# VUmcCGP/wisecondor

Measured on AMD Instinct MI355X. Metric: newref bin-pair distances/sec, higher is better.
Workload: dtype f64; 1 GPU; cfg2: newref 100 samples x 250 kb bins (11087 masked bins, refsize 100); parallelism=newref sharded by single rank, symmetric tiles, 1 rank(s), world_size=1

## Files before the change

### wisecondor_amd/csrc/ctx.h

```cpp
#pragma once
#include "common.h"

#define WC_MAX_CHROM 64

struct NewrefState {
    int64_t n_bins = 0, n_samples = 0;
    int64_t bins_pad = 0;
    int64_t k_pad16 = 0;
    int n_chrom = 0, k = 0, sum_order = 0;
    int64_t chrom_off[WC_MAX_CHROM + 1] = {0};
    const double *corrected = nullptr;
    int64_t n_sample_cols = 0;
    int64_t cap = 0;
    int64_t expect = 0;
    float beta = 0.f;
    bool prepared = false;
    double tau = 0.0;
    wc::DevBuf col_partial, col_mean, norm_lo, norm_hi, chrom_of_row, chrom_range, chrom_off_dev;
    wc::DevBuf sample_rows, sample_slot, s32, s_norm_lo, s_chrom, s_range, a16, s16;
    wc::DevBuf keys1, thr, cnt, list, tiles;
    wc::DevBuf fb_rows, fb_count, fb_scratch, stats, tiles0, pw_prog, pairs, x64, m2;
    bool fb_dirty = true;
    int64_t s_pad = 0;
    bool exact_only = false;
    wc::DevBuf cand_word;
    int index_bits = 17;
    int index_bits_req = 0;
    bool x64_pad = false;
    int pw_leaves = 0;
    int64_t pw_for = -1;
    std::vector<int64_t> sample_key, tiles0_key, tiles1_key, chrom_key;
    int64_t tiles0_n = 0, tiles1_n = 0;
};

struct TestState {
    std::vector<int> sel_host;
    wc::DevBuf counts, totals, raw, proj, data, xt, xc, zt, rt, nt, sdt, z, r, n, sd_avg;
    wc::DevBuf zc, rc, gpos, regions, sel;
    wc::DevBuf res_z, res_r, cwz, calls, n_calls;
    wc::DevBuf zs, rs2, ns2, sds, sub, tmin, tmax, tmin2, tmax2, cell_state, cell_rec, prefix, reg_abs, reg_flag, rs, jobs_a, jobs_b, job_cnt, partial, cbound, cuts, job_res, hot, cand, cand_cnt;
    wc::DevBuf seg, out_val, out_x, out_y, out_n, whole, effect, misc, misc2, reduce_tmp, win_bits, bit_off, pairs_a, pairs_b, cut_vals;
    wc::DevBuf walk_hot;
    int64_t rs_len = 0;
    hipGraphExec_t lat_exec = nullptr;
    std::vector<int64_t> lat_key, lat_fail_key;
    bool lat_warm = false;
    unsigned long long lat_epoch = 0;
    bool profile = false;
    std::vector<hipEvent_t> prof_ev;
    std::vector<int> prof_tag;
    wc::DevBuf sd_fail;
    wc::DevBuf prof_work;
    void mark(int tag, hipStream_t stream) {
        if (!profile) return;
        const size_t at = prof_tag.size();
        if (at >= prof_ev.size()) {
            hipEvent_t e = nullptr;
            if (hipEventCreate(&e) != hipSuccess) return;
            prof_ev.push_back(e);
        }
        if (hipEventRecord(prof_ev[at], stream) == hipSuccess) prof_tag.push_back(tag);
    }
};

struct PrepState {
    int64_t S = 0, Btot = 0, B = 0;
    bool ready = false;
    wc::DevBuf eig_ws;
};

struct ConvertState {
    wc::DevBuf tab, tiles, kpos, cls;
};

struct wc_ctx {
    int device = 0;
    PrepState prep;
    ConvertState cv;
    NewrefState nr;
    TestState ts;
    wc::DevBuf tmp_a, tmp_b, tmp_c, tmp_d;
    wc::DevBuf df_scratch, df_meta;
    wc::DevBuf js_slots, js_tiles;
    wc::DevBuf sp_plan;
    wc::DevBuf pl_list, pl_counts, pl_tab, pl_img, pl_part, pl_status;
    unsigned char *pl_host = nullptr;
    size_t pl_host_bytes = 0;
    hipEvent_t pl_sent = nullptr;
    int pl_host_reserve(size_t bytes) {
        if (!pl_sent) WC_HIP(hipEventCreateWithFlags(&pl_sent, hipEventDisableTiming));
        else WC_HIP(hipEventSynchronize(pl_sent));
        if (bytes <= pl_host_bytes) return WC_OK;
        if (pl_host) (void)hipHostFree(pl_host);
        pl_host = nullptr;
        pl_host_bytes = 0;
        const size_t ask = bytes + (bytes >> 1) + 256;
        WC_HIP(hipHostMalloc((void **)&pl_host, ask, hipHostMallocDefault));
        pl_host_bytes = ask;
        return WC_OK;
    }
    void *pinned = nullptr;
    size_t pinned_bytes = 0;
    int64_t last_stats[8] = {0};
    hipStream_t lat_stream = nullptr;
    hipEvent_t ev_lat_in = nullptr, ev_lat_out = nullptr;
// ... 73 lines not shown
```

### wisecondor_amd/csrc/newref.hip

```cpp
#include <cstring>
#include "ctx.h"

#include <algorithm>
#include <stdlib.h>

namespace {

constexpr int TB = 128;
constexpr int BK = 32;
constexpr int LDA = 36;
constexpr int LDT = 68;
constexpr int ROLE_ROWS = 1;
constexpr int ROLE_COLS = 2;
constexpr int MAX_SAMPLE_COLS = 4096;
constexpr int LIST_CAP = 1024;
constexpr int K_MAX = 1024;
constexpr int GL_ROW = 16;
constexpr int GL_STAGE = 2 * TB * GL_ROW;
#define WC_ADMIT_ALL FLT_MAX
constexpr double SENTINEL_DISTANCE = 1e10;

typedef float f32x16 __attribute__((ext_vector_type(16)));
typedef float f32x4 __attribute__((ext_vector_type(4)));
typedef _Float16 f16x8 __attribute__((ext_vector_type(8)));
// ... 2 lines not shown
typedef unsigned long long u64x2 __attribute__((ext_vector_type(2)));
typedef __attribute__((address_space(3))) void lds_void_t;
typedef __attribute__((address_space(1))) const void glb_void_t;
typedef __attribute__((address_space(3))) char lds_char_t;
typedef __attribute__((address_space(3))) f64x2 lds_f64x2_t;

__global__ __launch_bounds__(1024) void k_col_centre(const double *__restrict__ X, int64_t B, int64_t S,
                                                     int64_t n_rows, int64_t row_step,
                                                     double *__restrict__ centre, int *__restrict__ bad_norm) {
    __shared__ double sh_s[16][64];
    __shared__ double sh_c[16][64];
    __shared__ double sh_v[64];
    const int tx = threadIdx.x & 63, ty = threadIdx.x >> 6;
    const int64_t s = (int64_t)blockIdx.x * 64 + tx;
    if (blockIdx.x == 0 && threadIdx.x == 0) *bad_norm = 0x7F800000;
    constexpr int PER = 8;
    double val[PER];
#pragma unroll
    for (int e = 0; e < PER; ++e) {
        const int64_t q = ty + 16 * e;
        val[e] = (s < S && q < n_rows) ? X[(q * row_step) * S + s] : NAN;
    }
    double c = 0.0, rad = 0.0;
    for (int pass = 0; pass < 3; ++pass) {
        double sum = 0.0, cnt = 0.0;
#pragma unroll
        for (int e = 0; e < PER; ++e) {
            const double v = val[e];
            const bool ok = isfinite(v) && (pass != 2 || fabs(v - c) <= rad);
            sum += ok ? ((pass == 1) ? fabs(v - c) : v) : 0.0;
            cnt += ok ? 1.0 : 0.0;
        }
        sh_s[ty][tx] = sum;
        sh_c[ty][tx] = cnt;
        wc_sync();
        if (ty == 0) {
            double a = 0.0, b = 0.0;
            for (int r = 0; r < 16; ++r) { a += sh_s[r][tx]; b += sh_c[r][tx]; }
            sh_v[tx] = b > 0.0 ? a / b : 0.0;
        }
        wc_sync();
        if (pass == 0) c = sh_v[tx];
        else if (pass == 1) {
            rad = 8.0 * sh_v[tx];
            if (ty == 0 && s < S) centre[S + s] = sh_v[tx];
        } else if (ty == 0 && s < S) centre[s] = sh_v[tx];
        wc_sync();
    }
}

__device__ __host__ inline int64_t a16_index(int64_t row, int64_t s, int64_t Kpad16) {
    return (((row >> 7) * (Kpad16 >> 5) + (s >> 5)) << 12) + ((row & 127) << 5) + (s & 31);
}

__device__ inline unsigned short f32_to_f16_scaled(float a, double gam, double inv_gam, double &back, bool &clamped) {
    double sd = (double)a * gam;
    clamped = clamped || sd > 65504.0 || sd < -65504.0;
    sd = sd > 65504.0 ? 65504.0 : (sd < -65504.0 ? -65504.0 : sd);
    _Float16 h = (_Float16)(float)sd;
    if (fabs((double)(float)h) < 6.103515625e-05) h = (_Float16)0.f;
    back = (double)(float)h * inv_gam;
    unsigned short bits;
    __builtin_memcpy(&bits, &h, 2);
    return bits;
}

__host__ __device__ inline unsigned int slack_encode(float slack, int cb) {
    unsigned int u;
    __builtin_memcpy(&u, &slack, 4);
    u = u > 0x7F800000u ? 0x7F800000u : u;
    const int sh = 31 - cb;
    return (u + ((1u << sh) - 1u)) >> sh;
}
__host__ __device__ inline float slack_decode(unsigned int code, int cb) {
    const unsigned int u = code << (31 - cb);
    float f;
    __builtin_memcpy(&f, &u, 4);
    return f;
}
__device__ __forceinline__ float slack_of_word(unsigned int word, unsigned int index_mask) {
    return __uint_as_float((word >> 1) & ~(index_mask >> 1));
}

__global__ __launch_bounds__(256) void k_convert(const double *__restrict__ X, int64_t B, int64_t S,
                                                 int64_t Bpad,
                                                 const double *__restrict__ mean, double beta, double tau,
                                                 const int64_t *__restrict__ chrom_off, int n_chrom,
                                                 unsigned short *__restrict__ A16,
                                                 int64_t Kpad16, float *__restrict__ norm_lo,
                                                 float *__restrict__ norm_hi, int *__restrict__ chrom_of_row,
                                                 int2 *__restrict__ chrom_range,
                                                 const int *__restrict__ sample_slot,
                                                 unsigned short *__restrict__ S16, float *__restrict__ s_norm_lo,
                                                 int *__restrict__ s_chrom, int2 *__restrict__ s_range,
                                                 float *__restrict__ thr, int *__restrict__ cnt,
                                                 int *__restrict__ row_stat,
                                                 double *__restrict__ X64, int64_t Sp, float *__restrict__ m2_out,
                                                 int *__restrict__ bad_norm, int *__restrict__ fb_zero, int n_fb_zero,
                                                 unsigned int *__restrict__ cand_word, int index_bits) {
    const int lane = threadIdx.x & 63, hl = lane & 31, half = lane >> 5;
    const int64_t row = ((int64_t)blockIdx.x * 4 + (threadIdx.x >> 6)) * 2 + half;
    if (blockIdx.x == 0)
        for (int i = threadIdx.x; i < n_fb_zero; i += 256) fb_zero[i] = 0;
    if (row >= Bpad) return;
    constexpr int CB = 4;
    const int64_t xrow = (row < B ? row : 0) * S;
    auto load_x = [&](int64_t s0, double (&xv)[CB], double (&mv)[CB]) {
#pragma unroll
        for (int j = 0; j < CB; ++j) {
            const int64_t s = s0 + 32 * j, sc = s < S ? s : 0;
            xv[j] = X[xrow + sc];
            mv[j] = mean[sc];
        }
    };
    auto pin = [&](double (&v)[CB]) {
#pragma unroll
        for (int j = 0; j < CB; ++j) asm volatile("" : "+v"(v[j]));
    };
    auto load_scale = [&](int64_t s0, double (&sv)[CB]) {
#pragma unroll
        for (int j = 0; j < CB; ++j) {
            const int64_t s = s0 + 32 * j;
            sv[j] = mean[S + (s < S ? s : 0)];
        }
    };
    double xv[CB], mv[CB], sv[CB];
    load_scale(hl, sv);
    load_x(hl, xv, mv);
    int slot_w = sample_slot[row < B ? row : 0];
    int64_t end0_w = chrom_off[hl < n_chrom ? hl + 1 : 0], end1_w = chrom_off[hl + 32 < n_chrom ? hl + 33 : 0];
    asm volatile("" : "+v"(slot_w), "+v"(end0_w), "+v"(end1_w));
    pin(sv);
    pin(xv);
    pin(mv);
    const int slot = row < B ? slot_w : -1;
    int ch_w = -1;
    int2 range_w = make_int2(0, 0);
    {
        const int64_t none = (int64_t)0x7FFFFFFFFFFFFFFFll;
        const int64_t end0 = hl < n_chrom ? end0_w : none, end1 = hl + 32 < n_chrom ? end1_w : none;
        const unsigned long long b0 = __ballot(row < B && hl < n_chrom - 1 && row >= end0);
        const unsigned long long b1 = __ballot(row < B && hl + 32 < n_chrom - 1 && row >= end1);
        const int c = __popc((unsigned int)(b0 >> (32 * half))) + __popc((unsigned int)(b1 >> (32 * half)));
        auto end_of = [&](int i) {
            const int64_t a0 = __shfl(end0, (lane & 32) + (i & 31)), a1 = __shfl(end1, (lane & 32) + (i & 31));
            return i < 32 ? a0 : a1;
        };
        const int64_t e_lo = end_of(c ? c - 1 : 0), e_hi = end_of(c);
        if (row < B) {
            ch_w = c;
            range_w = make_int2((int)(c ? e_lo : 0), (int)e_hi);
        }
    }
    double gam = 1.0, inv_gam = 1.0;
    {
        double t = 0.0, c = 0.0;
        for (int64_t s0 = hl; s0 < S; s0 += 32 * CB) {
            if (s0 != hl) { load_scale(s0, sv); pin(sv); }
#pragma unroll
            for (int j = 0; j < CB; ++j) {
                const double m = sv[j];
                if (s0 + 32 * j < S && isfinite(m) && m > 0.0) { t += m; c += 1.0; }
            }
        }
        for (int o = 16; o > 0; o >>= 1) { t += __shfl_xor(t, o); c += __shfl_xor(c, o); }
        if (c > 0.0 && isfinite(t)) {
            int e = ilogb(t / c);
            e = e < -60 ? -60 : (e > 60 ? 60 : e);
            gam = ldexp(1.0, 2 - e);
            inv_gam = ldexp(1.0, e - 2);
        }
        if (row == 0 && hl == 0) *m2_out = (float)(-2.0 * inv_gam * inv_gam);
    }
    double acc = 0.0, e2 = 0.0, hn = 0.0;
    bool clamped = false;
    for (int64_t s0 = hl; s0 < Kpad16; s0 += 32 * CB) {
        if (s0 != hl) { load_x(s0, xv, mv); pin(xv); pin(mv); }
#pragma unroll
        for (int j = 0; j < CB; ++j) {
            const int64_t s = s0 + 32 * j;
            if (s < Kpad16) {
                if (X64 && row < B && s < Sp) X64[row * Sp + s] = s < S ? xv[j] : 0.0;
                float a = 0.f;
                if (row < B && s < S) a = (float)(xv[j] - mv[j]);
                double back;
                const unsigned short h = f32_to_f16_scaled(a, gam, inv_gam, back, clamped);
                const double err = (double)a - back;
                e2 += err * err;
                hn += back * back;
                A16[a16_index(row, s, Kpad16)] = h;
                if (slot >= 0) S16[(int64_t)slot * Kpad16 + s] = h;
                acc += (double)a * (double)a;
            }
        }
    }
    for (int o = 16; o > 0; o >>= 1) {
        acc += __shfl_xor(acc, o);
        e2 += __shfl_xor(e2, o);
        hn += __shfl_xor(hn, o);
    }
    clamped = ((unsigned int)(__ballot(clamped) >> (32 * half))) != 0u;
    if (hl == 0) {
        float lo = INFINITY, hi = INFINITY;
        int ch = -1;
        int2 range = make_int2(0, 0);
        if (row < B) {
            if (isfinite(acc) && acc < 1e37 && isfinite(e2) && isfinite(hn) && clamped) {
                atomicMin(bad_norm, __float_as_int(__double2float_rd(sqrt(acc) * (1.0 - 1e-6))));
            } else if (isfinite(acc) && acc < 1e37 && isfinite(e2) && isfinite(hn)) {
                const double m = fmax(acc, hn);
                lo = __double2float_rd(acc - (e2 / tau + tau * m) * (1.0 + 1e-9) - beta * m - 1e-37);
                hi = __double2float_ru(2.0 * (acc - (double)lo) * (1.0 + 1e-6) + 1e-37);
            }
            ch = ch_w;
            range = range_w;
        }
        chrom_range[row] = range;
        norm_lo[row] = lo;
        norm_hi[row] = hi;
        cand_word[row] = (unsigned int)row | (slack_encode(hi, 32 - index_bits) << index_bits);
        chrom_of_row[row] = ch;
        if (slot >= 0) {
            s_norm_lo[slot] = lo;
            s_chrom[slot] = ch;
            s_range[slot] = range;
        }
        thr[row] = -INFINITY;
        cnt[row] = 0;
        row_stat[row] = (int)0xFEFEFEFE;
    }
}

__global__ void k_pad_samples(int64_t Kpad16, int64_t first, unsigned short *__restrict__ S16,
                              float *__restrict__ s_norm_lo, int *__restrict__ s_chrom,
                              int2 *__restrict__ s_range) {
    int64_t m = first + blockIdx.x;
    for (int64_t s = threadIdx.x; s < Kpad16; s += blockDim.x) S16[m * Kpad16 + s] = (unsigned short)0;
    if (threadIdx.x == 0) {
        s_norm_lo[m] = INFINITY;
        s_chrom[m] = -2;
        s_range[m] = make_int2(0, 0);
    }
}


struct GramArgs {
    const float *P, *Q;
    int64_t ld;
    const float *m2;
    int nslab32, last_steps32;
    const float *nbP, *nbQ;
    const unsigned int *cwP, *cwQ;
    const int2 *range;
    const int4 *tiles;
    int ntiles;
    const float *thr;
    int *cnt;
    unsigned long long *list;
    int cap;
};

__device__ inline unsigned int key_code16(float key) {
    const unsigned int code = __float_as_uint(fmaxf(key, 0.f)) >> 15;
    return key < INFINITY ? code : 0xFFFFu;
}
__device__ inline float key_from_code16(unsigned int code) {
    return __uint_as_float((code << 15) | 0x7FFFu);
}

__device__ inline unsigned int run_mask(int a, int b) {
    a = a < 0 ? 0 : a;
    b = b > 32 ? 32 : b;
    if (a >= b) return 0u;
    const unsigned int upto_b = b == 32 ? ~0u : ((1u << b) - 1u);
    return upto_b & ~((1u << a) - 1u);
}

__device__ inline unsigned long long pack_passed(float key, unsigned int word) {
    const unsigned int b = __float_as_uint(key);
    return ((unsigned long long)((b & 0x80000000u) ? ~b : (b | 0x80000000u)) << 32) | word;
}

__device__ __forceinline__ void shift_in_le(unsigned int &mask, float key, float thr) {
    asm("v_cmp_le_f32 vcc, %1, %2\n\tv_addc_co_u32 %0, vcc, %0, %0, vcc" : "+v"(mask) : "v"(key), "v"(thr) : "vcc");
}

__device__ inline void wave_lds_fence() {
    __builtin_amdgcn_fence(__ATOMIC_RELEASE, "wavefront");
    __builtin_amdgcn_wave_barrier();
    __builtin_amdgcn_fence(__ATOMIC_ACQUIRE, "wavefront");
}

__device__ inline unsigned long long pack_entry(float key, int j) {
    return ((unsigned long long)wc::f32_ordered(key) << 32) | (unsigned int)j;
}


constexpr int EP_LD = 32;
constexpr int EP_BLOCK = 64 * EP_LD;
constexpr int EP_MASKS = 128;
static_assert(4 * EP_BLOCK <= 2 * GL_STAGE, "the four dot blocks alias the two operand stages");

__device__ __forceinline__ int ep_at(int col, int row) {
    return col * EP_LD + ((((row >> 2) ^ col) & 7) << 2) + (row & 3);
}

__device__ __forceinline__ void gram_epilogue(const GramArgs &g, float *sm, const float *nbPs, const float *nbQs,
                                              const float *thPs, const float *thQs, const unsigned int *cwPs,
                                              const unsigned int *cwQs, f32x16 (&acc)[2][2], const int I,
                                              const int J, const int roles, const float m2, const int lane, const int w,
                                              const int wr, const int wc, const int li, const int lh) {
    __builtin_amdgcn_s_setprio(0);
    const int row0 = I * TB + wr * 64, col0 = J * TB + wc * 64;
    const int2 rgq0 = g.range[(int64_t)col0 + li], rgq1 = g.range[(int64_t)col0 + 32 + li];
    const int2 rgr = g.range[(int64_t)row0 + lane];
// ... 1706 lines not shown
                 (long long)st.bins_pad, need);
        st.index_bits = st.index_bits_req ? st.index_bits_req : std::min(24, std::max(17, need));
    }
    st.k_pad16 = round_up(n_samples, 64);
    st.cap = LIST_CAP;
    st.expect = LIST_CAP * 3 / 8;
    const double chain = (double)(n_samples + 16) * 5.9604644775390625e-08;
    st.beta = (float)(2.0 * chain * 1.001);
    st.tau = 2.44140625e-04;
    int64_t M = round_up((n_bins + 13) / 14, TB);
    if (M < 512) M = 512;
    if (M > MAX_SAMPLE_COLS) M = MAX_SAMPLE_COLS;
    if (M > st.bins_pad) M = st.bins_pad;
    st.n_sample_cols = M;

    int rc;
    if ((rc = st.col_mean.reserve(sizeof(double) * 3 * n_samples))) return rc;
    st.s_pad = round_up(n_samples, 16);
    st.x64_pad = n_samples <= 2048 && st.bins_pad * st.s_pad * 8 < (1ll << 32);
    if (st.x64_pad && (rc = st.x64.reserve(sizeof(double) * st.bins_pad * st.s_pad))) return rc;
    if ((rc = st.m2.reserve(sizeof(float) * 4))) return rc;
    if ((rc = st.norm_lo.reserve(sizeof(float) * st.bins_pad))) return rc;
    if ((rc = st.norm_hi.reserve(sizeof(float) * st.bins_pad))) return rc;
    if ((rc = st.cand_word.reserve(sizeof(unsigned int) * st.bins_pad))) return rc;
    if ((rc = st.chrom_of_row.reserve(sizeof(int) * st.bins_pad))) return rc;
    if ((rc = st.chrom_range.reserve(sizeof(int2) * st.bins_pad))) return rc;
    if ((rc = st.chrom_off_dev.reserve(sizeof(int64_t) * (WC_MAX_CHROM + 1)))) return rc;
    if ((rc = st.sample_rows.reserve(sizeof(int) * M))) return rc;
    if ((rc = st.sample_slot.reserve(sizeof(int) * st.bins_pad))) return rc;
    if ((rc = st.a16.reserve(sizeof(unsigned short) * st.bins_pad * st.k_pad16))) return rc;
    if ((rc = st.s16.reserve(sizeof(unsigned short) * M * st.k_pad16))) return rc;
    if ((rc = st.s_norm_lo.reserve(sizeof(float) * M))) return rc;
    if ((rc = st.s_chrom.reserve(sizeof(int) * M))) return rc;
    if ((rc = st.s_range.reserve(sizeof(int2) * M))) return rc;
    if ((rc = st.keys1.reserve(sizeof(unsigned short) * st.bins_pad * M))) return rc;
    if ((rc = st.thr.reserve(sizeof(float) * st.bins_pad))) return rc;
    if ((rc = st.cnt.reserve(sizeof(int) * st.bins_pad))) return rc;
    if ((rc = st.list.reserve(sizeof(uint64_t) * st.bins_pad * st.cap))) return rc;
    if ((rc = st.fb_rows.reserve(sizeof(int) * st.bins_pad))) return rc;
    if ((rc = st.fb_count.reserve(sizeof(int) * 4))) return rc;
    if ((rc = st.stats.reserve(sizeof(int) * st.bins_pad))) return rc;

    {
        std::vector<int64_t> ckey(st.chrom_off, st.chrom_off + n_chrom + 1);
        if (ckey != st.chrom_key) {
            WC_HIP(hipMemcpyAsync(st.chrom_off_dev.p, st.chrom_off, sizeof(int64_t) * (n_chrom + 1),
                                  hipMemcpyHostToDevice, stream));
            WC_HIP(hipStreamSynchronize(stream));
            st.chrom_key = ckey;
        }
    }
    if (st.pw_for != n_samples) {
        std::vector<int2> prog;
        build_pairwise_leaves((int)n_samples, 0, prog);
        if ((rc = st.pw_prog.reserve(sizeof(int2) * prog.size()))) return rc;
        WC_HIP(hipMemcpyAsync(st.pw_prog.p, prog.data(), sizeof(int2) * prog.size(), hipMemcpyHostToDevice, stream));
        WC_HIP(hipStreamSynchronize(stream));
        st.pw_leaves = (int)prog.size();
        st.pw_for = n_samples;
    }
    std::vector<int64_t> skey = {n_bins, M};
    if (skey != st.sample_key) {
        int64_t real = std::min<int64_t>(M, n_bins);
        std::vector<int> perm(n_bins);
        for (int64_t i = 0; i < n_bins; ++i) perm[i] = (int)i;
        uint64_t s = 0x9E3779B97F4A7C15ull;
        for (int64_t i = 0; i < real; ++i) {
            s = s * 6364136223846793005ull + 1442695040888963407ull;
            int64_t pick = i + (int64_t)((s >> 33) % (uint64_t)(n_bins - i));
            std::swap(perm[i], perm[pick]);
        }
        std::sort(perm.begin(), perm.begin() + real);
        std::vector<int> slot((size_t)n_bins, -1);
        for (int64_t i = 0; i < real; ++i) slot[perm[i]] = (int)i;
        WC_HIP(hipMemcpyAsync(st.sample_rows.p, perm.data(), sizeof(int) * real, hipMemcpyHostToDevice, stream));
        WC_HIP(hipMemcpyAsync(st.sample_slot.p, slot.data(), sizeof(int) * n_bins, hipMemcpyHostToDevice, stream));
        WC_HIP(hipStreamSynchronize(stream));
        st.sample_key = skey;
        st.tiles0_key.clear();
        st.tiles1_key.clear();
    }

    double *mean2 = st.col_mean.as<double>();
    {
        int64_t n_rows = std::min<int64_t>(n_bins, 128);
        int64_t row_step = n_bins / n_rows;
        hipLaunchKernelGGL(k_col_centre, dim3((unsigned)((n_samples + 63) / 64)), dim3(1024), 0, stream, corrected,
                           n_bins, n_samples, n_rows, row_step, mean2, st.m2.as<int>() + 1);
    }

    hipLaunchKernelGGL(k_convert, dim3((unsigned)(st.bins_pad / 8)), dim3(256), 0, stream, corrected, n_bins,
                       n_samples, st.bins_pad, (const double *)mean2, (double)st.beta, st.tau,
                       st.chrom_off_dev.as<int64_t>(), n_chrom, st.a16.as<unsigned short>(),
                       st.k_pad16, st.norm_lo.as<float>(), st.norm_hi.as<float>(), st.chrom_of_row.as<int>(),
                       st.chrom_range.as<int2>(), (const int *)st.sample_slot.as<int>(),
                       st.s16.as<unsigned short>(), st.s_norm_lo.as<float>(), st.s_chrom.as<int>(),
                       st.s_range.as<int2>(), st.thr.as<float>(), st.cnt.as<int>(), st.stats.as<int>(),
                       st.x64_pad ? st.x64.as<double>() : (double *)nullptr, st.s_pad, st.m2.as<float>(),
                       st.m2.as<int>() + 1, st.fb_count.as<int>(), 4, st.cand_word.as<unsigned int>(), st.index_bits);
    st.fb_dirty = false;
    if (M > n_bins)
        hipLaunchKernelGGL(k_pad_samples, dim3((unsigned)(M - n_bins)), dim3(256), 0, stream, st.k_pad16, n_bins,
                           st.s16.as<unsigned short>(), st.s_norm_lo.as<float>(), st.s_chrom.as<int>(),
                           st.s_range.as<int2>());
    WC_HIP(hipGetLastError());
    st.prepared = true;
    return WC_OK;
}

int wc_newref_thresholds_dev(wc_ctx *ctx, void *stream_, int64_t row_begin, int64_t row_end) {
    WC_CHECK(ctx && ctx->nr.prepared, WC_E_ARG, "newref: prepare has not run");
    NewrefState &st = ctx->nr;
    WC_CHECK(row_begin >= 0 && row_begin <= row_end && row_end <= st.n_bins, WC_E_ARG, "newref: bad row range");
    if (row_begin == row_end || st.exact_only) return WC_OK;
    hipStream_t stream = (hipStream_t)stream_;
    const int ib = (int)(row_begin / TB), ie = (int)((row_end + TB - 1) / TB);
    const int mb = (int)(st.n_sample_cols / TB);
    std::vector<int64_t> key = {st.bins_pad, st.n_sample_cols, ib, ie};
    if (key != st.tiles0_key) {
        std::vector<int4> tiles;
        tiles.reserve((size_t)(ie - ib) * mb);
        for (int I = ib; I < ie; ++I)
            for (int J = 0; J < mb; ++J) tiles.push_back(make_int4(I, J, 0, 0));
        int rc;
        if ((rc = st.tiles0.reserve(sizeof(int4) * tiles.size()))) return rc;
        WC_HIP(hipMemcpyAsync(st.tiles0.p, tiles.data(), sizeof(int4) * tiles.size(), hipMemcpyHostToDevice, stream));
        WC_HIP(hipStreamSynchronize(stream));
        st.tiles0_key = key;
        st.tiles0_n = (int64_t)tiles.size();
    }
    {
        const int ntiles = (int)st.tiles0_n;
        unsigned grid = (unsigned)(((ntiles + 7) / 8) * 8);
        hipLaunchKernelGGL(k_gram_thr16, dim3(grid), dim3(256), 0, stream,
                           (const unsigned short *)st.a16.as<unsigned short>(),
                           (const unsigned short *)st.s16.as<unsigned short>(), st.k_pad16, (int)(st.k_pad16 / 64),
                           (const float *)st.norm_lo.as<float>(), (const float *)st.s_norm_lo.as<float>(),
                           (const int2 *)st.s_range.as<int2>(), (const int4 *)st.tiles0.as<int4>(), ntiles,
                           st.keys1.as<unsigned int>(), st.n_sample_cols, (const float *)st.m2.as<float>());
    }
    unsigned sg = (unsigned)((row_end - row_begin + 3) / 4);
    {
        const unsigned int *kp = st.keys1.as<unsigned int>();
        const int2 *cr = st.chrom_range.as<int2>();
        const int per_lane = (int)(st.n_sample_cols / 64);
#define WC_SELECT(NV)                                                                                          \
    hipLaunchKernelGGL(k_select_thr<NV>, dim3(sg), dim3(256), 0, stream, kp, st.n_sample_cols,                \
                       (int)st.n_sample_cols, cr, st.n_bins, row_begin, row_end, (int)st.expect, (int)st.cap, \
                       st.thr.as<float>())
        if (per_lane <= 16) WC_SELECT(16);
        else if (per_lane <= 32) WC_SELECT(32);
        else WC_SELECT(64);
#undef WC_SELECT
    }
    WC_HIP(hipGetLastError());
    return WC_OK;
}

int64_t wc_newref_list_capacity(wc_ctx *ctx) { return ctx ? ctx->nr.cap : 0; }

int wc_newref_get_thresholds_dev(wc_ctx *ctx, void *stream, int64_t row_begin, int64_t row_end, float *out) {
    WC_CHECK(ctx && ctx->nr.prepared && out, WC_E_ARG, "newref: bad argument");
    WC_CHECK(row_begin >= 0 && row_begin <= row_end && row_end <= ctx->nr.n_bins, WC_E_ARG, "newref: bad row range");
    if (row_end > row_begin)
        WC_HIP(hipMemcpyAsync(out, ctx->nr.thr.as<float>() + row_begin, sizeof(float) * (row_end - row_begin),
                              hipMemcpyDeviceToDevice, (hipStream_t)stream));
    return WC_OK;
}

int wc_newref_get_bounds_dev(wc_ctx *ctx, void *stream, int64_t row_begin, int64_t row_end, float *lo_out,
                             float *slack_out) {
    WC_CHECK(ctx && ctx->nr.prepared && lo_out && slack_out, WC_E_ARG, "newref: bad argument");
    WC_CHECK(row_begin >= 0 && row_begin <= row_end && row_end <= ctx->nr.n_bins, WC_E_ARG, "newref: bad row range");
    if (row_end > row_begin) {
        WC_HIP(hipMemcpyAsync(lo_out, ctx->nr.norm_lo.as<float>() + row_begin, sizeof(float) * (row_end - row_begin),
                              hipMemcpyDeviceToDevice, (hipStream_t)stream));
        WC_HIP(hipMemcpyAsync(slack_out, ctx->nr.norm_hi.as<float>() + row_begin, sizeof(float) * (row_end - row_begin),
                              hipMemcpyDeviceToDevice, (hipStream_t)stream));
    }
    return WC_OK;
}

// ... 54 lines not shown
                               const int32_t *src_cnt, const uint64_t *src_list) {
    WC_CHECK(ctx && ctx->nr.prepared && src_cnt && src_list && src_cap > 0, WC_E_ARG, "newref: bad argument");
    WC_CHECK(row_begin >= 0 && row_begin <= row_end && row_end <= ctx->nr.n_bins, WC_E_ARG, "newref: bad row range");
    if (row_end == row_begin) return WC_OK;
    NewrefState &st = ctx->nr;
    hipLaunchKernelGGL(k_import_lists, dim3((unsigned)(row_end - row_begin)), dim3(64), 0, (hipStream_t)stream,
                       st.cnt.as<int>(), st.list.as<unsigned long long>(), (int)st.cap, row_begin, (int)src_cap,
                       src_cnt, (const unsigned long long *)src_list,
                       (const unsigned int *)st.cand_word.as<unsigned int>(), (1u << st.index_bits) - 1u,
                       (unsigned int)st.bins_pad);
    WC_HIP(hipGetLastError());
    return WC_OK;
}

int wc_newref_collect_dev(wc_ctx *ctx, void *stream_, int64_t row_begin, int64_t row_end, int tile_rank,
                          int tile_ranks) {
    WC_CHECK(ctx && ctx->nr.prepared, WC_E_ARG, "newref: prepare has not run");
    NewrefState &st = ctx->nr;
    WC_CHECK(row_begin >= 0 && row_begin <= row_end && row_end <= st.n_bins, WC_E_ARG, "newref: bad row range");
    WC_CHECK(tile_ranks >= 1 && tile_rank >= 0 && tile_rank < tile_ranks, WC_E_ARG, "newref: bad tile rank");
    if (row_begin == row_end || st.exact_only) return WC_OK;
    hipStream_t stream = (hipStream_t)stream_;
    std::vector<int64_t> key = {st.n_bins, row_begin, row_end, tile_rank, tile_ranks};
    for (int c = 0; c <= st.n_chrom; ++c) key.push_back(st.chrom_off[c]);
    if (key != st.tiles1_key) {
        std::vector<int4> tiles;
        build_tiles(st, row_begin, row_end, tile_rank, tile_ranks, tiles);
        int rc;
        if ((rc = st.tiles.reserve(sizeof(int4) * std::max<size_t>(tiles.size(), 1)))) return rc;
        if (!tiles.empty()) {
            WC_HIP(hipMemcpyAsync(st.tiles.p, tiles.data(), sizeof(int4) * tiles.size(), hipMemcpyHostToDevice, stream));
            WC_HIP(hipStreamSynchronize(stream));
        }
        st.tiles1_key = key;
        st.tiles1_n = (int64_t)tiles.size();
    }
    ctx->last_stats[2] = st.tiles1_n;
    ctx->last_stats[3] = st.n_sample_cols;
    if (st.tiles1_n == 0) return WC_OK;
    GramArgs g{};
    g.P = g.Q = st.a16.as<float>();
    g.ld = st.k_pad16 / 2;
    g.m2 = st.m2.as<float>();
    g.nslab32 = (int)((st.n_samples + 31) / 32);
    g.last_steps32 = (int)(((st.n_samples - (int64_t)(g.nslab32 - 1) * 32) + 15) / 16);
    g.nbP = g.nbQ = st.norm_lo.as<float>();
    g.cwP = g.cwQ = st.cand_word.as<unsigned int>();
    g.range = st.chrom_range.as<int2>();
    g.tiles = st.tiles.as<int4>();
    g.ntiles = (int)st.tiles1_n;
    g.thr = st.thr.as<float>();
    g.cnt = st.cnt.as<int>();
    g.list = st.list.as<unsigned long long>();
    g.cap = (int)st.cap;
    const unsigned grid = (unsigned)(((g.ntiles + 7) / 8) * 8);
    hipLaunchKernelGGL(k_gram_glds, dim3(grid), dim3(256), 0, stream, g);
    WC_HIP(hipGetLastError());
    return WC_OK;
}

static void finish_args(NewrefState &st, int64_t row_begin, int64_t row_end, int32_t *idx_out, double *dist_out,
                        FinishArgs &a) {
    a.X = st.corrected;
    a.B = st.n_bins;
    a.S = st.n_samples;
    a.norm_lo = st.norm_lo.as<float>();
    a.norm_hi = st.norm_hi.as<float>();
    a.thr = st.thr.as<float>();
    a.cnt = st.cnt.as<int>();
    a.list = st.list.as<unsigned long long>();
    a.index_mask = (1u << st.index_bits) - 1u;
    a.cap = (int)st.cap;
    a.k = st.k;
    a.beta = (double)st.beta;
    a.chrom_of_row = st.chrom_of_row.as<int>();
    a.chrom_off = st.chrom_off_dev.as<int64_t>();
    a.chrom_range = st.chrom_range.as<int2>();
    a.row_begin = row_begin;
    a.row_end = row_end;
    a.idx_out = idx_out;
    a.dist_out = dist_out;
    a.fb_rows = st.fb_rows.as<int>();
    a.fb_count = st.fb_count.as<int>();
    a.bad_norm = st.m2.as<float>() + 1;
    a.row_stat = st.stats.as<int>();
    a.sum_order = st.sum_order;
    a.lone_mask = 0ull;
    if (st.sum_order == WC_SUM_SEQUENTIAL)
        for (int c = 0; c < st.n_chrom; ++c)
            if (st.chrom_off[c] <= 1 && st.n_bins - st.chrom_off[c + 1] <= 1) a.lone_mask |= 1ull << c;
    a.xs_in_lds = st.n_samples <= 2048;
    a.pw_prog = st.pw_prog.as<int2>();
    a.pw_leaves = st.pw_leaves;
}

static int launch_exact(NewrefState &st, hipStream_t stream, const FinishArgs &a, int64_t n_host) {
    int rc;
    const int cap = n_host < 0 ? EX_DEV_CAP : EX_CAP;
    if ((rc = st.fb_scratch.reserve(sizeof(uint64_t) * (n_host < 0 ? 2 : 1) * cap * st.bins_pad))) return rc;
    const bool seq = st.sum_order == WC_SUM_SEQUENTIAL || st.n_samples < 8;
    const int edge = seq ? 64 : 32;
    const unsigned ctiles = (unsigned)((st.n_bins + edge - 1) / edge);
    unsigned long long *scratch = st.fb_scratch.as<unsigned long long>();
    const int *rows = st.fb_rows.as<int>();
    if (n_host < 0) {
        const int rgroups = 4;
        int *sync = st.fb_count.as<int>() + 1;
        constexpr int EXD_TILE_WGS = 192, EXD_SEL_WGS = 64;
        const int n_tile = (int)std::min<int64_t>((int64_t)ctiles * rgroups, EXD_TILE_WGS);
        const unsigned grid = (unsigned)(n_tile + EXD_SEL_WGS);
        if (seq) hipLaunchKernelGGL((k_exact_dev<true>), dim3(grid), dim3(256), 0, stream, a, rows,
                                    (const int *)st.fb_count.as<int>(), sync, scratch, st.bins_pad, cap, (int)ctiles, rgroups, EXD_SEL_WGS);
        else hipLaunchKernelGGL((k_exact_dev<false>), dim3(grid), dim3(256), 0, stream, a, rows,
                                (const int *)st.fb_count.as<int>(), sync, scratch, st.bins_pad, cap, (int)ctiles, rgroups, EXD_SEL_WGS);
        return WC_OK;
    }
    for (int64_t first = 0; first < n_host; first += cap) {
        const int64_t nf = std::min<int64_t>(cap, n_host - first);
        const unsigned rgroups = (unsigned)((nf + edge - 1) / edge);
        if (seq) hipLaunchKernelGGL((k_exact_tile<true>), dim3(ctiles, rgroups), dim3(256), 0, stream, a, rows,
                                    (const int *)nullptr, (int)n_host, (int)first, scratch, st.bins_pad, cap);
        else hipLaunchKernelGGL((k_exact_tile<false>), dim3(ctiles, rgroups), dim3(256), 0, stream, a, rows,
                                (const int *)nullptr, (int)n_host, (int)first, scratch, st.bins_pad, cap);
        hipLaunchKernelGGL(k_exact_select, dim3((unsigned)nf), dim3(256), 0, stream, a, rows, (int)n_host, (int)first,
                           scratch, st.bins_pad, cap);
    }
    return WC_OK;
}

static int newref_finish_part(wc_ctx *ctx, void *stream_, int64_t row_begin, int64_t row_end, int32_t *idx_out,
                              double *dist_out, int which) {
    WC_CHECK(ctx && ctx->nr.prepared, WC_E_ARG, "newref: prepare has not run");
    NewrefState &st = ctx->nr;
    WC_CHECK(row_begin >= 0 && row_begin <= row_end && row_end <= st.n_bins, WC_E_ARG, "newref: bad row range");
    WC_CHECK(idx_out && dist_out, WC_E_ARG, "newref: NULL output");
    if (row_begin == row_end) return WC_OK;
    hipStream_t stream = (hipStream_t)stream_;
    int rc;
    if (which & 5) {
        if (st.fb_dirty) WC_HIP(hipMemsetAsync(st.fb_count.p, 0, sizeof(int) * 4, stream));
        st.fb_dirty = true;
    }
    FinishArgs a{};
    finish_args(st, row_begin, row_end, idx_out, dist_out, a);
    const int ps = (int)std::max<int64_t>(128, std::min<int64_t>(PS_MAX, round_up(st.k + 28, 64)));
    const bool pair_engine = st.x64_pad && !st.exact_only;
    if ((which & 12) && !pair_engine) which = (which & ~12) | ((which & 4) ? 1 : 0);
    const bool seq = st.sum_order == WC_SUM_SEQUENTIAL || st.n_samples < 8;
    const unsigned rows = (unsigned)(row_end - row_begin);
    if ((which & 1) && st.exact_only) {
        hipLaunchKernelGGL(k_all_exact, dim3((rows + 255) / 256), dim3(256), 0, stream, a);
    } else if ((which & 13) && pair_engine) {
        if ((rc = st.pairs.reserve(sizeof(int) * st.bins_pad * RMAX))) return rc;
        PickArgs p{a, st.pairs.as<int>(), ps};
        if (which & 5) hipLaunchKernelGGL(k_pick, dim3((rows + 3) / 4), dim3(256), 0, stream, p);
        const size_t slabs = sizeof(double) * (size_t)(ps / 64) * SLAB_DOUBLES;
        const size_t order = (sizeof(unsigned long long) + sizeof(int)) * (2 * RMAX + 4);
        const size_t dyn = sizeof(double) * st.s_pad + std::max(slabs, order);
        if (!(which & 9)) {
        } else if (seq) hipLaunchKernelGGL((k_rescore<true, false>), dim3(rows), dim3(ps), dyn, stream, p,
                                           (const double *)st.x64.as<double>(), (int)st.s_pad);
        else hipLaunchKernelGGL((k_rescore<false, true>), dim3(rows), dim3(ps), dyn, stream, p,
                                (const double *)st.x64.as<double>(), (int)st.s_pad);
    } else if (which & 1) {
        const size_t dyn = a.xs_in_lds ? sizeof(double) * st.n_samples : 0;
        if (seq) hipLaunchKernelGGL((k_finish<true, 128>), dim3(rows), dim3(128), dyn, stream, a);
        else hipLaunchKernelGGL((k_finish<false, 128>), dim3(rows), dim3(128), dyn, stream, a);
// ... 143 lines not shown
```

Before: 740.0 billion bin-pair distances/s.

## Fuse column centring into convert kernel with per-block LDS centre/scale

```diff
diff --git a/wisecondor_amd/csrc/ctx.h b/wisecondor_amd/csrc/ctx.h
--- a/wisecondor_amd/csrc/ctx.h
+++ b/wisecondor_amd/csrc/ctx.h
@@ -21,6 +21,8 @@
     wc::DevBuf keys1, thr, cnt, list, tiles;
     wc::DevBuf fb_rows, fb_count, fb_scratch, stats, tiles0, pw_prog, pairs, x64, m2;
     bool fb_dirty = true;
+    int bad_slot = 0;
+    bool bad_spare_clean = false;
     int64_t s_pad = 0;
     bool exact_only = false;
     wc::DevBuf cand_word;
diff --git a/wisecondor_amd/csrc/newref.hip b/wisecondor_amd/csrc/newref.hip
--- a/wisecondor_amd/csrc/newref.hip
+++ b/wisecondor_amd/csrc/newref.hip
@@ -108,28 +108,27 @@
     return __uint_as_float((word >> 1) & ~(index_mask >> 1));
 }
 
-__global__ __launch_bounds__(256) void k_convert(const double *__restrict__ X, int64_t B, int64_t S,
-                                                 int64_t Bpad,
-                                                 const double *__restrict__ mean, double beta, double tau,
-                                                 const int64_t *__restrict__ chrom_off, int n_chrom,
-                                                 unsigned short *__restrict__ A16,
-                                                 int64_t Kpad16, float *__restrict__ norm_lo,
-                                                 float *__restrict__ norm_hi, int *__restrict__ chrom_of_row,
-                                                 int2 *__restrict__ chrom_range,
-                                                 const int *__restrict__ sample_slot,
-                                                 unsigned short *__restrict__ S16, float *__restrict__ s_norm_lo,
-                                                 int *__restrict__ s_chrom, int2 *__restrict__ s_range,
-                                                 float *__restrict__ thr, int *__restrict__ cnt,
-                                                 int *__restrict__ row_stat,
-                                                 double *__restrict__ X64, int64_t Sp, float *__restrict__ m2_out,
-                                                 int *__restrict__ bad_norm, int *__restrict__ fb_zero, int n_fb_zero,
-                                                 unsigned int *__restrict__ cand_word, int index_bits) {
+template <bool CENTRE_IN_LDS, int NT>
+__device__ __forceinline__ void convert_row(const double *__restrict__ X, int64_t B, int64_t S, int64_t Bpad,
+                                            const double *mean, double beta, double tau,
+                                            const int64_t *__restrict__ chrom_off, int n_chrom,
+                                            unsigned short *__restrict__ A16, int64_t Kpad16,
+                                            float *__restrict__ norm_lo, float *__restrict__ norm_hi,
+                                            int *__restrict__ chrom_of_row, int2 *__restrict__ chrom_range,
+                                            const int *__restrict__ sample_slot, unsigned short *__restrict__ S16,
+                                            float *__restrict__ s_norm_lo, int *__restrict__ s_chrom,
+                                            int2 *__restrict__ s_range, float *__restrict__ thr, int *__restrict__ cnt,
+                                            int *__restrict__ row_stat, double *__restrict__ X64, int64_t Sp,
+                                            float *__restrict__ m2_out, int *__restrict__ bad_norm,
+                                            int *__restrict__ fb_zero, int n_fb_zero,
+                                            unsigned int *__restrict__ cand_word, int index_bits) {
     const int lane = threadIdx.x & 63, hl = lane & 31, half = lane >> 5;
-    const int64_t row = ((int64_t)blockIdx.x * 4 + (threadIdx.x >> 6)) * 2 + half;
+    const int64_t row = ((int64_t)blockIdx.x * (NT / 64) + (threadIdx.x >> 6)) * 2 + half;
     if (blockIdx.x == 0)
-        for (int i = threadIdx.x; i < n_fb_zero; i += 256) fb_zero[i] = 0;
+        for (int i = threadIdx.x; i < n_fb_zero; i += NT) fb_zero[i] = 0;
     if (row >= Bpad) return;
     constexpr int CB = 4;
+    const int64_t scale_off = CENTRE_IN_LDS ? 128 : S;
     const int64_t xrow = (row < B ? row : 0) * S;
     auto load_x = [&](int64_t s0, double (&xv)[CB], double (&mv)[CB]) {
 #pragma unroll
@@ -147,7 +146,7 @@
 #pragma unroll
         for (int j = 0; j < CB; ++j) {
             const int64_t s = s0 + 32 * j;
-            sv[j] = mean[S + (s < S ? s : 0)];
+            sv[j] = mean[scale_off + (s < S ? s : 0)];
         }
     };
     double xv[CB], mv[CB], sv[CB];
@@ -257,6 +256,88 @@
     }
 }
 
+#define WC_CONVERT_PARAMS                                                                                            \
+    const double *__restrict__ X, int64_t B, int64_t S, int64_t Bpad, const double *__restrict__ mean, double beta, \
+        double tau, const int64_t *__restrict__ chrom_off, int n_chrom, unsigned short *__restrict__ A16,           \
+        int64_t Kpad16, float *__restrict__ norm_lo, float *__restrict__ norm_hi, int *__restrict__ chrom_of_row,   \
+        int2 *__restrict__ chrom_range, const int *__restrict__ sample_slot, unsigned short *__restrict__ S16,      \
+        float *__restrict__ s_norm_lo, int *__restrict__ s_chrom, int2 *__restrict__ s_range,                       \
+        float *__restrict__ thr, int *__restrict__ cnt, int *__restrict__ row_stat, double *__restrict__ X64,       \
+        int64_t Sp, float *__restrict__ m2_out, int *__restrict__ bad_norm, int *__restrict__ fb_zero,              \
+        int n_fb_zero, unsigned int *__restrict__ cand_word, int index_bits
+#define WC_CONVERT_ARGS(mean_)                                                                                        \
+    X, B, S, Bpad, mean_, beta, tau, chrom_off, n_chrom, A16, Kpad16, norm_lo, norm_hi, chrom_of_row, chrom_range,   \
+        sample_slot, S16, s_norm_lo, s_chrom, s_range, thr, cnt, row_stat, X64, Sp, m2_out, bad_norm, fb_zero,       \
+        n_fb_zero, cand_word, index_bits
+
+__global__ __launch_bounds__(256) void k_convert(WC_CONVERT_PARAMS) {
+    convert_row<false, 256>(WC_CONVERT_ARGS(mean));
+}
+
+constexpr int FUSED_CENTRE_ROWS = 32;
+constexpr int FUSED_MAX_SAMPLES = 128;
+constexpr int FUSED_THREADS = 512;
+constexpr int FUSED_WGS_PER_CU = 3;
+template <int CR, int NT>
+__global__ __launch_bounds__(NT, FUSED_WGS_PER_CU) void k_prepare_fused(WC_CONVERT_PARAMS, double *__restrict__ mean_out,
+                                                                       int64_t n_crows, int64_t crow_step,
+                                                                       int *__restrict__ bad_spare) {
+    constexpr int NPH = NT / 128, PER = CR / NPH;
+    static_assert(CR % NPH == 0, "whole rows per phase");
+    __shared__ float sh_part[2][2][NPH][128];
+    __shared__ double sh_cs[2 * 128];
+    const int tx = threadIdx.x & 127, ty = __builtin_amdgcn_readfirstlane(threadIdx.x >> 7);
+    if (blockIdx.x == 0 && threadIdx.x == 0) *bad_spare = 0x7F800000;
+    double val[PER];
+    {
+        const unsigned int sc = tx < S ? tx : 0;
+#pragma unroll
+        for (int e = 0; e < PER; ++e) {
+            const int64_t q = ty + NPH * e;
+            const double *__restrict__ xq = X + ((q < n_crows ? q : 0) * crow_step) * S;
+            val[e] = xq[sc];
+        }
+    }
+#pragma unroll
+    for (int e = 0; e < PER; ++e) asm volatile("" : "+v"(val[e]));
+    float fv[PER];
+#pragma unroll
+    for (int e = 0; e < PER; ++e) fv[e] = (tx < S && ty + NPH * e < n_crows) ? (float)val[e] : NAN;
+    float c = 0.f, rad = 0.f, mad = 0.f;
+    for (int pass = 0; pass < 3; ++pass) {
+        float sum = 0.f, n = 0.f;
+#pragma unroll
+        for (int e = 0; e < PER; ++e) {
+            const float v = fv[e];
+            const bool ok = isfinite(v) && (pass != 2 || fabsf(v - c) <= rad);
+            sum += ok ? ((pass == 1) ? fabsf(v - c) : v) : 0.f;
+            n += ok ? 1.f : 0.f;
+        }
+        float (*part)[NPH][128] = sh_part[pass & 1];
+        part[0][ty][tx] = sum;
+        part[1][ty][tx] = n;
+        wc_sync();
+        float a = 0.f, b = 0.f;
+#pragma unroll
+        for (int r = 0; r < NPH; ++r) { a += part[0][r][tx]; b += part[1][r][tx]; }
+        const float v = b > 0.f ? a / b : 0.f;
+        if (pass == 1) { mad = v; rad = 8.f * v; }
+        else c = v;
+    }
+    if (ty == 0) {
+        sh_cs[tx] = (double)c;
+        sh_cs[128 + tx] = (double)mad;
+        if (blockIdx.x == 0 && tx < S) {
+            mean_out[tx] = (double)c;
+            mean_out[S + tx] = (double)mad;
+        }
+    }
+    wc_sync();
+    convert_row<true, NT>(WC_CONVERT_ARGS((const double *)sh_cs));
+}
+#undef WC_CONVERT_PARAMS
+#undef WC_CONVERT_ARGS
+
 __global__ void k_pad_samples(int64_t Kpad16, int64_t first, unsigned short *__restrict__ S16,
                               float *__restrict__ s_norm_lo, int *__restrict__ s_chrom,
                               int2 *__restrict__ s_range) {
@@ -2129,22 +2210,42 @@
     }
 
     double *mean2 = st.col_mean.as<double>();
-    {
+    if (n_samples <= FUSED_MAX_SAMPLES) {
+        const int slot = 1 - st.bad_slot;
+        int *bad = st.m2.as<int>() + 1 + slot, *spare = st.m2.as<int>() + 1 + st.bad_slot;
+        if (!st.bad_spare_clean) WC_HIP(hipMemsetD32Async((hipDeviceptr_t)bad, 0x7F800000, 1, stream));
+        const int64_t n_crows = std::min<int64_t>(n_bins, FUSED_CENTRE_ROWS);
+        const int64_t crow_step = n_bins >= 128 ? (128 / FUSED_CENTRE_ROWS) * (n_bins / 128) : n_bins / n_crows;
+        hipLaunchKernelGGL((k_prepare_fused<FUSED_CENTRE_ROWS, FUSED_THREADS>),
+                           dim3((unsigned)(st.bins_pad / (FUSED_THREADS / 32))), dim3(FUSED_THREADS),
+                           0, stream, corrected, n_bins, n_samples, st.bins_pad, (const double *)nullptr,
+                           (double)st.beta, st.tau, st.chrom_off_dev.as<int64_t>(), n_chrom,
+                           st.a16.as<unsigned short>(), st.k_pad16, st.norm_lo.as<float>(), st.norm_hi.as<float>(),
+                           st.chrom_of_row.as<int>(), st.chrom_range.as<int2>(),
+                           (const int *)st.sample_slot.as<int>(), st.s16.as<unsigned short>(),
+                           st.s_norm_lo.as<float>(), st.s_chrom.as<int>(), st.s_range.as<int2>(), st.thr.as<float>(),
+                           st.cnt.as<int>(), st.stats.as<int>(), st.x64_pad ? st.x64.as<double>() : (double *)nullptr,
+                           st.s_pad, st.m2.as<float>(), bad, st.fb_count.as<int>(), 4,
+                           st.cand_word.as<unsigned int>(), st.index_bits, mean2, n_crows, crow_step, spare);
+        WC_HIP(hipGetLastError());
+        st.bad_slot = slot;
+        st.bad_spare_clean = true;
+    } else {
         int64_t n_rows = std::min<int64_t>(n_bins, 128);
         int64_t row_step = n_bins / n_rows;
+        int *bad = st.m2.as<int>() + 1 + st.bad_slot;
         hipLaunchKernelGGL(k_col_centre, dim3((unsigned)((n_samples + 63) / 64)), dim3(1024), 0, stream, corrected,
-                           n_bins, n_samples, n_rows, row_step, mean2, st.m2.as<int>() + 1);
-    }
-
-    hipLaunchKernelGGL(k_convert, dim3((unsigned)(st.bins_pad / 8)), dim3(256), 0, stream, corrected, n_bins,
-                       n_samples, st.bins_pad, (const double *)mean2, (double)st.beta, st.tau,
-                       st.chrom_off_dev.as<int64_t>(), n_chrom, st.a16.as<unsigned short>(),
-                       st.k_pad16, st.norm_lo.as<float>(), st.norm_hi.as<float>(), st.chrom_of_row.as<int>(),
-                       st.chrom_range.as<int2>(), (const int *)st.sample_slot.as<int>(),
-                       st.s16.as<unsigned short>(), st.s_norm_lo.as<float>(), st.s_chrom.as<int>(),
-                       st.s_range.as<int2>(), st.thr.as<float>(), st.cnt.as<int>(), st.stats.as<int>(),
-                       st.x64_pad ? st.x64.as<double>() : (double *)nullptr, st.s_pad, st.m2.as<float>(),
-                       st.m2.as<int>() + 1, st.fb_count.as<int>(), 4, st.cand_word.as<unsigned int>(), st.index_bits);
+                           n_bins, n_samples, n_rows, row_step, mean2, bad);
+        hipLaunchKernelGGL(k_convert, dim3((unsigned)(st.bins_pad / 8)), dim3(256), 0, stream, corrected, n_bins,
+                           n_samples, st.bins_pad, (const double *)mean2, (double)st.beta, st.tau,
+                           st.chrom_off_dev.as<int64_t>(), n_chrom, st.a16.as<unsigned short>(),
+                           st.k_pad16, st.norm_lo.as<float>(), st.norm_hi.as<float>(), st.chrom_of_row.as<int>(),
+                           st.chrom_range.as<int2>(), (const int *)st.sample_slot.as<int>(),
+                           st.s16.as<unsigned short>(), st.s_norm_lo.as<float>(), st.s_chrom.as<int>(),
+                           st.s_range.as<int2>(), st.thr.as<float>(), st.cnt.as<int>(), st.stats.as<int>(),
+                           st.x64_pad ? st.x64.as<double>() : (double *)nullptr, st.s_pad, st.m2.as<float>(),
+                           bad, st.fb_count.as<int>(), 4, st.cand_word.as<unsigned int>(), st.index_bits);
+    }
     st.fb_dirty = false;
     if (M > n_bins)
         hipLaunchKernelGGL(k_pad_samples, dim3((unsigned)(M - n_bins)), dim3(256), 0, stream, st.k_pad16, n_bins,
@@ -2365,7 +2466,7 @@
     a.dist_out = dist_out;
     a.fb_rows = st.fb_rows.as<int>();
     a.fb_count = st.fb_count.as<int>();
-    a.bad_norm = st.m2.as<float>() + 1;
+    a.bad_norm = st.m2.as<float>() + 1 + st.bad_slot;
     a.row_stat = st.stats.as<int>();
     a.sum_order = st.sum_order;
     a.lone_mask = 0ull;
```

Measured after the change: 753.4 billion bin-pair distances/s (median of 6 runs). 1.8% higher.
